# NVIDIA-ISAAC-ROS/isaac_ros_nvblox

Measured on NVIDIA H100. Metric: depth-frames/sec (TSDF+ESDF integrate, 640x480 @ 5 cm voxels), higher is better.
Workload: dtype f32

## Files before the change

### isaac_ros_nvblox_b200/csrc/nvb_api.cu

```cuda
#include <algorithm>
#include <array>
#include <cfloat>
#include <cmath>
#include <cstdio>
#include <cstring>
#include <functional>
#include <set>
#include <string>
#include <vector>

#include "nvb_internal.cuh"

using namespace nvb;

namespace {

thread_local std::string g_last_error;

int fail(int code, const std::string& msg) {
  g_last_error = msg;
  return code;
}

#define NVB_CUDA(expr)                                                                               \
// ... 992 lines not shown
      launchEsdfSliceAllocateAndMark(c, from_tracker ? nullptr : in_xyz_dev, todo.slots, todo.count,
                                     from_tracker ? upper : n_explicit, m->num_sms, st);
      m->launches += 3;
    } else {
      launchEsdfAllocate(c, from_tracker ? nullptr : in_xyz_dev, todo.slots, todo.count, from_tracker ? upper : n_explicit, st);
      launchEsdfMark(c, upper, m->num_sms, st);
      m->launches += 2;
    }
  };
  if (m->esdf_persistent) {
    cudaStream_t es = m->esdf_stream;
    NVB_CUDA(cudaEventRecord(m->esdf_ready, m->stream));
    NVB_CUDA(cudaStreamWaitEvent(es, m->esdf_ready, 0));
    beginStageOn(m, 3, es);
    allocAndMark(es);
    endStageOn(m, es);
    NVB_CUDA(cudaEventRecord(m->mark_done, es));
    NVB_CUDA(cudaStreamWaitEvent(m->stream, m->mark_done, 0));
    beginStageOn(m, 4, es);
    launchEsdfClear(c, m->esdf.capacity, m->num_sms, es);
    m->launches++;
    endStageOn(m, es);
    beginStageOn(m, 5, es);
    e = m->esdf_persistent == 3   ? launchEsdfComputeX(c, m->num_sms, m->esdf_reserved_sms, es, &launches)
        : m->esdf_persistent == 2 ? launchEsdfComputeGes(c, m->num_sms, es, &launches)
                                  : launchEsdfComputePersistent(c, m->num_sms, es, &launches);
    endStageOn(m, es);
    if (e == cudaSuccess) {
      NVB_CUDA(cudaEventRecord(m->esdf_done, es));
      m->esdf_in_flight = true;
    }
  } else {
    NVB_CUDA(joinEsdf(m));
    beginStage(m, 3);
    allocAndMark(m->stream);
    endStage(m);
    beginStage(m, 4);
    launchEsdfClear(c, m->esdf.capacity, m->num_sms, m->stream);
    m->launches++;
    endStage(m);
    beginStage(m, 5);
    e = runEsdfComputeHostLoop(c, m->num_sms, m->stream, &launches);
    endStage(m);
  }
  m->launches += launches;
  if (e != cudaSuccess) return fail(NVB_ERR_CUDA, std::string("ESDF compute launch: ") + cudaGetErrorString(e));
  return NVB_OK;
}

}

extern "C" {

const char* nvb_last_error(void) { return g_last_error.c_str(); }
const char* nvb_version(void) { return "nvblox_b200 0.1 (sm_90a)"; }

int32_t nvb_device_count(void) {
  int n = 0;
  if (cudaGetDeviceCount(&n) != cudaSuccess) {
    cudaGetLastError();
    return 0;
  }
  return n;
}

void nvb_default_mapper_options(NvbMapperOptions* o) {
  if (!o) return;
  o->voxel_size_m = 0.05f;
  o->device = 0;
  o->tsdf_capacity_blocks = kDefaultCapacity;
  o->esdf_capacity_blocks = kDefaultCapacity;
  o->esdf_persistent = 3;
  o->projective_layer_type = NVB_PROJECTIVE_TSDF;
  o->keep_last_view = 0;
}
void nvb_default_tsdf_params(NvbTsdfParams* p) {
  if (!p) return;
  memset(p, 0, sizeof(*p));
  p->truncation_distance_vox = 4.0f;
  p->max_integration_distance_m = 7.0f;
  p->max_weight = 5.0f;
  p->invalid_depth_decay_factor = -1.0f;
  p->weighting_type = NVB_WEIGHT_INVERSE_SQUARE;
  p->raycast_subsampling = 4;
  p->workspace_bounds_type = NVB_WS_UNBOUNDED;
}
void nvb_default_esdf_params(NvbEsdfParams* p) {
  if (!p) return;
  p->max_esdf_distance_m = 2.0f;
  p->max_site_distance_vox = 1.0f;
  p->min_weight = 1e-4f;
  p->occupied_threshold = 0.5f;
}
void nvb_default_occupancy_params(NvbOccupancyParams* p) {
  if (!p) return;
  p->free_region_occupancy_probability = 0.3f;
  p->occupied_region_occupancy_probability = 0.7f;
  p->unobserved_region_occupancy_probability = 0.5f;
  p->occupied_region_half_width_m = 0.1f;
}

static int createMapperResources(const NvbMapperOptions* opts, NvbMapper* m) {
  m->device = opts->device;
  cudaDeviceProp prop;
  NVB_CUDA(cudaGetDeviceProperties(&prop, opts->device));
  m->num_sms = prop.multiProcessorCount;
  m->voxel_size = opts->voxel_size_m;
  m->block_size = opts->voxel_size_m * (float)kVps;
  nvb_default_tsdf_params(&m->tp);
  nvb_default_esdf_params(&m->ep);
  nvb_default_occupancy_params(&m->op);
  nvb_default_tsdf_decay_params(&m->tdp);
  nvb_default_occupancy_decay_params(&m->odp);
  nvb_default_freespace_params(&m->fp);
  nvb_default_esdf_slice_params(&m->sp);
  nvb_default_color_params(&m->cp);
  nvb_default_ground_plane_params(&m->gp);
  m->projective_layer_type = opts->projective_layer_type;
  m->keep_last_view = opts->keep_last_view ? 1 : 0;
  m->esdf_persistent = opts->esdf_persistent;
  m->esdf_split_min_k = esdfWaveXSplitMinK();
  if (const char* e = getenv("NVB_GES_SWITCH")) m->ges_switch = atoi(e);
  {
    const char* e = getenv("NVB_CLEAR_PRUNE");
    m->prune_default = m->esdf_persistent == 3 && !(e && atoi(e) == 0);
    m->prune_ok = m->prune_default;
  }
  NVB_CUDA(cudaStreamCreateWithFlags(&m->stream, cudaStreamNonBlocking));
  NVB_CUDA(cudaStreamCreateWithFlags(&m->copy_stream, cudaStreamNonBlocking));
  {
    int lo = 0, hi = 0;
    cudaDeviceGetStreamPriorityRange(&lo, &hi);
    NVB_CUDA(cudaStreamCreateWithPriority(&m->esdf_stream, cudaStreamNonBlocking, hi));
  }
  NVB_CUDA(cudaEventCreateWithFlags(&m->esdf_ready, cudaEventDisableTiming));
  NVB_CUDA(cudaEventCreateWithFlags(&m->esdf_done, cudaEventDisableTiming));
  NVB_CUDA(cudaEventCreateWithFlags(&m->mark_done, cudaEventDisableTiming));
  const int tcap = opts->tsdf_capacity_blocks > 0 ? opts->tsdf_capacity_blocks : kDefaultCapacity;
  const int ecap = std::max(opts->esdf_capacity_blocks > 0 ? opts->esdf_capacity_blocks : kDefaultCapacity, tcap);
  int rc;
  if ((rc = allocLayer(&m->tsdf, tcap, m->projective_layer_type == NVB_PROJECTIVE_OCCUPANCY ? kOccBlockBytes : kTsdfBlockBytes,
                       m->stream))) return rc;
  if ((rc = allocLayer(&m->esdf, ecap, kEsdfBlockBytes, m->stream))) return rc;
  if (m->projective_layer_type == NVB_PROJECTIVE_TSDF_WITH_FREESPACE &&
      (rc = allocLayer(&m->freespace, tcap, kFreespaceBlockBytes, m->stream)))
    return rc;
  NVB_CUDA(m->esdf_ints.grow(m, kNumInts, kNumInts, 0));
  if ((rc = growTracker(m, tcap))) return rc;
  if ((rc = allocEsdfScratch(m, ecap))) return rc;
  const int one = 1;
  NVB_CUDA(cudaMemcpyAsync(m->esdf_ints.get() + kRingId, &one, sizeof(int), cudaMemcpyHostToDevice, m->stream));
  m->frame_count = m->esdf_ints.get() + kFrameCount;
  m->error_dev = m->esdf_ints.get() + kError;
  NVB_CUDA(m->clr_bits.grow(m, 2048, 2048));
  NVB_CUDA(m->stats.grow(m, 16, 16, 0));
  NVB_CUDA(m->phase_max.grow(m, 4000, 4000, 0));
  NVB_CUDA(m->barrier.grow(m, 16, 16, 0));
  NVB_CUDA(m->ticket.grow(m, 16, 16, 0));
  NVB_CUDA(cudaMallocHost(&m->h_ints, 64 * sizeof(int)));
  memset(m->h_ints, 0, 64 * sizeof(int));
  NVB_CUDA(cudaMallocHost(&m->h_list, (size_t)kHostListCap * sizeof(int4)));
  NVB_CUDA(cudaMallocHost(&m->h_count_ring, kCountRing * sizeof(int)));
  for (int k = 0; k < kCountRing; k++) {
    NVB_CUDA(cudaEventCreateWithFlags(&m->count_events[k], cudaEventDisableTiming));
    m->count_pending[k] = false;
    m->count_cum_at[k] = 0;
  }
  for (int k = 0; k < kStagingBuffers; k++) {
    NVB_CUDA(cudaEventCreateWithFlags(&m->stage_copied[k], cudaEventDisableTiming));
    NVB_CUDA(cudaEventCreateWithFlags(&m->stage_consumed[k], cudaEventDisableTiming));
  }
  NVB_CUDA(syncAll(m));
  return NVB_OK;
}

int32_t nvb_mapper_create(const NvbMapperOptions* opts, NvbMapper** out) {
  if (!opts || !out) return fail(NVB_ERR_INVALID_ARGUMENT, "null argument");
  if (!(opts->voxel_size_m > 0.0f)) return fail(NVB_ERR_INVALID_ARGUMENT, "voxel_size_m must be > 0");
  int ndev = 0;
  if (cudaGetDeviceCount(&ndev) != cudaSuccess || ndev == 0) {
    cudaGetLastError();
    return fail(NVB_ERR_NO_DEVICE, "no CUDA device: the depth-integration path has no CPU fallback");
  }
  if (opts->device < 0 || opts->device >= ndev) return fail(NVB_ERR_INVALID_ARGUMENT, "bad device ordinal");
  if (opts->projective_layer_type != NVB_PROJECTIVE_TSDF && opts->projective_layer_type != NVB_PROJECTIVE_OCCUPANCY &&
      opts->projective_layer_type != NVB_PROJECTIVE_TSDF_WITH_FREESPACE)
    return fail(NVB_ERR_INVALID_ARGUMENT, "unknown projective_layer_type");
  NVB_CUDA(cudaSetDevice(opts->device));
  NvbMapper* m = new NvbMapper();
  const int rc = createMapperResources(opts, m);
  if (rc != NVB_OK) {
    const std::string why = g_last_error;
    nvb_mapper_destroy(m);
    cudaGetLastError();
    g_last_error = why;
    return rc;
  }
  *out = m;
  return NVB_OK;
}

void nvb_mapper_destroy(NvbMapper* m) {
  if (!m) return;
  cudaSetDevice(m->device);
  syncAll(m);
  cudaStreamSynchronize(m->copy_stream);
  collectStages(m);
  cudaEventDestroy(m->esdf_ready), cudaEventDestroy(m->esdf_done), cudaEventDestroy(m->mark_done);
  cudaStreamDestroy(m->esdf_stream);
  freeLayer(&m->tsdf), freeLayer(&m->esdf);
  if (m->freespace.blocks) freeLayer(&m->freespace);
  if (m->color.blocks) freeLayer(&m->color);
  for (int k = 0; k < kStagingBuffers; k++) {
    cudaEventDestroy(m->stage_copied[k]), cudaEventDestroy(m->stage_consumed[k]);
  }
  if (m->dyn_event) cudaEventDestroy(m->dyn_event);
  if (m->query_event) cudaEventDestroy(m->query_event);
  if (m->mesh.blocks) freeLayer(&m->mesh);
  cudaFreeHost(m->h_ints), cudaFreeHost(m->h_count_ring), cudaFreeHost(m->h_list);
  for (int k = 0; k < kCountRing; k++) cudaEventDestroy(m->count_events[k]);
  cudaStreamDestroy(m->stream), cudaStreamDestroy(m->copy_stream);
  delete m;
}

static int resetLayers(NvbMapper* m) {
  NVB_CUDA(syncAll(m));
  std::vector<DevLayer*> layers = {&m->tsdf, &m->esdf};
  if (m->freespace.blocks) layers.push_back(&m->freespace);
  if (m->color.blocks) layers.push_back(&m->color);
  for (DevLayer* L : layers) {
    int count = 0;
    NVB_CUDA(cudaMemcpy(&count, L->count, sizeof(int), cudaMemcpyDeviceToHost));
    count = std::min(count, L->capacity);
    NVB_CUDA(cudaMemsetAsync(L->blocks, 0, (size_t)count * L->block_bytes, m->stream));
    NVB_CUDA(cudaMemsetAsync(L->count, 0, sizeof(int), m->stream));
    NVB_CUDA(cudaMemsetAsync(L->free_count, 0, sizeof(int), m->stream));
    launchFillU64(L->hash.keys, kEmptyKey, (size_t)L->hash.mask + 1, m->stream);
  }
  int rc;
  if ((rc = resetTracker(m))) return rc;
  NVB_CUDA(cudaMemsetAsync(m->esdf_ints.get() + kClearedCount, 0, sizeof(int), m->stream));
  NVB_CUDA(cudaMemsetAsync(m->esdf_ints.get() + kClearedSeq, 0, sizeof(int), m->stream));
  NVB_CUDA(cudaMemsetAsync(m->esdf_ints.get() + kDeadClearedCount, 0, sizeof(int), m->stream));
  NVB_CUDA(cudaMemsetAsync(m->seed_upd.get(), 0, (size_t)m->esdf.capacity * sizeof(int), m->stream));
  NVB_CUDA(cudaMemsetAsync(m->seed_clr.get(), 0, (size_t)m->esdf.capacity * sizeof(int), m->stream));
  NVB_CUDA(cudaMemsetAsync(m->psum.get(), 0, 2 * (size_t)m->esdf.capacity * sizeof(int), m->stream));
  m->prune_ok = m->prune_default;
  NVB_CUDA(cudaMemsetAsync(m->nbr.get(), 0xFE, (size_t)m->esdf.capacity * 6 * sizeof(int), m->stream));
  NVB_CUDA(cudaMemsetAsync(m->nbr27.get(), 0xFE, (size_t)m->esdf.capacity * 27 * sizeof(int), m->stream));
  NVB_CUDA(cudaMemsetAsync(m->error_dev, 0, sizeof(int), m->stream));
  if (m->mesh.blocks) {
    NVB_CUDA(cudaMemsetAsync(m->mesh.blocks, 0, (size_t)m->mesh.capacity * m->mesh.block_bytes, m->stream));
    NVB_CUDA(cudaMemsetAsync(m->mesh.count, 0, sizeof(int), m->stream));
    NVB_CUDA(cudaMemsetAsync(m->mesh.free_count, 0, sizeof(int), m->stream));
    launchFillU64(m->mesh.hash.keys, kEmptyKey, (size_t)m->mesh.hash.mask + 1, m->stream);
    NVB_CUDA(cudaMemsetAsync(m->mesh_state.get(), 0, kArenaInts * sizeof(int), m->stream));
  }
  m->tsdf_count_ub = 0, m->tsdf_count_confirmed = 0, m->esdf_extra_ub = 0;
  m->cells_cum = 0, m->confirmed_cum = 0;
  for (int k = 0; k < kCountRing; k++) m->count_pending[k] = false;
  NVB_CUDA(syncAll(m));
  return NVB_OK;
}

int32_t nvb_mapper_clear(NvbMapper* m) {
  if (!m) return fail(NVB_ERR_INVALID_ARGUMENT, "null mapper");
  NVB_CUDA(cudaSetDevice(m->device));
  const int rc = resetLayers(m);
  if (rc) return rc;
  m->esdf_mode = 0;
  m->fs_last_update_ms = 0;
  m->has_last_view = false;
  return NVB_OK;
}

int32_t nvb_mapper_set_tsdf_params(NvbMapper* m, const NvbTsdfParams* p) {
  if (!m || !p) return fail(NVB_ERR_INVALID_ARGUMENT, "null argument");
  if (!(p->max_weight > 0.0f)) return fail(NVB_ERR_INVALID_ARGUMENT, "max_weight must be > 0");
  if (!(p->truncation_distance_vox > 0.0f)) return fail(NVB_ERR_INVALID_ARGUMENT, "truncation_distance_vox must be > 0");
  if (p->raycast_subsampling < 1) return fail(NVB_ERR_INVALID_ARGUMENT, "raycast_subsampling must be >= 1");
  if (p->weighting_type < 0 || p->weighting_type > NVB_WEIGHT_LINEAR_WITH_MAX)
    return fail(NVB_ERR_INVALID_ARGUMENT, "unknown weighting_type");
  if (p->workspace_bounds_type < 0 || p->workspace_bounds_type > NVB_WS_BOUNDING_BOX)
    return fail(NVB_ERR_INVALID_ARGUMENT, "unknown workspace_bounds_type");
  m->tp = *p;
  return NVB_OK;
}
int32_t nvb_mapper_get_tsdf_params(const NvbMapper* m, NvbTsdfParams* p) {
  if (!m || !p) return fail(NVB_ERR_INVALID_ARGUMENT, "null argument");
  *p = m->tp;
  return NVB_OK;
}
int32_t nvb_mapper_set_esdf_params(NvbMapper* m, const NvbEsdfParams* p) {
  if (!m || !p) return fail(NVB_ERR_INVALID_ARGUMENT, "null argument");
  if (!(p->max_esdf_distance_m > 0.0f) || !(p->max_site_distance_vox > 0.0f) || !(p->min_weight > 0.0f))
    return fail(NVB_ERR_INVALID_ARGUMENT, "ESDF parameters must be > 0");
  if (!(p->occupied_threshold >= 0.0f && p->occupied_threshold <= 1.0f))
    return fail(NVB_ERR_INVALID_ARGUMENT, "occupied_threshold must be a probability");
  m->ep = *p;
  return NVB_OK;
}
int32_t nvb_mapper_get_esdf_params(const NvbMapper* m, NvbEsdfParams* p) {
  if (!m || !p) return fail(NVB_ERR_INVALID_ARGUMENT, "null argument");
  *p = m->ep;
  return NVB_OK;
}
int32_t nvb_mapper_set_occupancy_params(NvbMapper* m, const NvbOccupancyParams* p) {
// ... 2306 lines not shown
```

### isaac_ros_nvblox_b200/csrc/nvb_esdf.cu

```cuda
#include "nvb_esdf_common.cuh"
#include "nvb_tma.cuh"

#include <cstdlib>

namespace nvb {

namespace {

constexpr int kClearBitWords = 2048;
__device__ __forceinline__ int clearBitWord(int x, int y) { return ((x & 63) << 5) | (y & 31); }

__device__ __forceinline__ void resetEsdfUpdate(const EsdfCtx& c, int n) {
  const int i = blockIdx.x * blockDim.x + threadIdx.x;
  if (i == 0) {
    *c.work_count = n;
    *c.upd_count = 0;
    *c.clr_count = 0;
    c.clr_aabb[0] = c.clr_aabb[1] = c.clr_aabb[2] = INT32_MAX;
    c.clr_aabb[3] = c.clr_aabb[4] = c.clr_aabb[5] = INT32_MIN;
    c.ring_count[0] = c.ring_count[1] = 0;
    c.ring_count[2] = 0;
    c.ges_counts[0] = c.ges_counts[1] = c.ges_counts[2] = c.ges_counts[3] = 0;
    *c.barrier = 0;
    for (int k = 0; k < 16; k++) c.stats[k] = 0;
    c.stats[0] = n;
  }
  for (int q = i; q < 4000; q += gridDim.x * blockDim.x) c.phase_max[q] = 0ull;
  if (c.clr_bits)
    for (int q = i; q < kClearBitWords; q += gridDim.x * blockDim.x) c.clr_bits[q] = 0u;
}

__global__ void esdfAllocateKernel(EsdfCtx c, const int* in_xyz, const int* in_slots, const int* in_count_dev,
                                   int in_count_host) {
  const int n = in_count_dev ? *in_count_dev : in_count_host;
  const int i = blockIdx.x * blockDim.x + threadIdx.x;
  resetEsdfUpdate(c, n);
  if (i >= n) return;
  int x, y, z, tslot;
  if (in_slots) {
    tslot = in_slots[i];
    if (c.tracker_dirty) c.tracker_dirty[tslot] = 0;
    x = c.tsdf.block_index[3 * tslot], y = c.tsdf.block_index[3 * tslot + 1], z = c.tsdf.block_index[3 * tslot + 2];
  } else {
    x = in_xyz[3 * i], y = in_xyz[3 * i + 1], z = in_xyz[3 * i + 2];
    tslot = hashFind(c.tsdf.hash, x, y, z);
  }
  bool was_new;
  const int eslot = hashFindOrInsert(c.esdf, x, y, z, c.error, &was_new);
  const int fslot = c.use_freespace ? hashFind(c.freespace.hash, x, y, z) : -1;
  c.work[i] = make_int4(eslot, tslot, was_new ? 1 : 0, fslot);
}

constexpr int kMarkLocalMax = 64;
struct MarkLocal {
  int upd[kMarkLocalMax];
  int clr[kMarkLocalMax];
  int nu, nc;
  int aabb[6];
};
__device__ __forceinline__ void markLocalInit(MarkLocal& ml) {
  ml.nu = ml.nc = 0;
  ml.aabb[0] = ml.aabb[1] = ml.aabb[2] = INT32_MAX;
  ml.aabb[3] = ml.aabb[4] = ml.aabb[5] = INT32_MIN;
}
__device__ __forceinline__ void markLocalFlush(const EsdfCtx& c, MarkLocal& ml) {
  if (ml.nu) {
    const int base = atomicAdd(c.upd_count, ml.nu);
    for (int i = 0; i < ml.nu; i++) c.upd_list[base + i] = ml.upd[i];
  }
  if (ml.nc) {
    const int base = atomicAdd(c.clr_count, ml.nc);
    for (int i = 0; i < ml.nc; i++) c.clr_list[base + i] = ml.clr[i];
    atomicMin(c.clr_aabb + 0, ml.aabb[0]), atomicMin(c.clr_aabb + 1, ml.aabb[1]), atomicMin(c.clr_aabb + 2, ml.aabb[2]);
    atomicMax(c.clr_aabb + 3, ml.aabb[3]), atomicMax(c.clr_aabb + 4, ml.aabb[4]), atomicMax(c.clr_aabb + 5, ml.aabb[5]);
  }
  markLocalInit(ml);
}
__device__ __forceinline__ void markLocalRecord(const EsdfCtx& c, MarkLocal& ml, int slot, bool updated, bool cleared,
                                                const int* bi_known = nullptr) {
  if (updated) {
    if (ml.nu == kMarkLocalMax) markLocalFlush(c, ml);
    ml.upd[ml.nu++] = slot;
    c.seed_upd[slot] = c.update_seq;
  }
  if (cleared) {
    if (ml.nc == kMarkLocalMax) markLocalFlush(c, ml);
    ml.clr[ml.nc++] = slot;
    const int* bi = bi_known ? bi_known : c.esdf.block_index + 3 * slot;
    const int x = bi[0], y = bi[1], z = bi[2];
    ml.aabb[0] = min(ml.aabb[0], x), ml.aabb[1] = min(ml.aabb[1], y), ml.aabb[2] = min(ml.aabb[2], z);
    ml.aabb[3] = max(ml.aabb[3], x), ml.aabb[4] = max(ml.aabb[4], y), ml.aabb[5] = max(ml.aabb[5], z);
    if (c.clr_bits) atomicOr(c.clr_bits + clearBitWord(x, y), 1u << (z & 31));
  }
}

__device__ __forceinline__ void updatePersistentClearedList(const EsdfCtx& c, int nclr) {
  if (nclr > 0) {
    *c.cleared_count = 0;
    *c.cleared_seq = c.update_seq;
    if (c.dead_cleared_count) *c.dead_cleared_count = 0;
    return;
  }
  if (!c.dead_cleared_count) return;
  int nd = *c.dead_cleared_count;
  for (int i = 0; i < nd;) {
    const int slot = hashFind(c.esdf.hash, c.dead_cleared_xyz[3 * i], c.dead_cleared_xyz[3 * i + 1], c.dead_cleared_xyz[3 * i + 2]);
    if (slot >= 0) {
      c.cleared_list[(*c.cleared_count)++] = slot;
      c.seed_clr[slot] = *c.cleared_seq;
      nd--;
      c.dead_cleared_xyz[3 * i] = c.dead_cleared_xyz[3 * nd], c.dead_cleared_xyz[3 * i + 1] = c.dead_cleared_xyz[3 * nd + 1],
                          c.dead_cleared_xyz[3 * i + 2] = c.dead_cleared_xyz[3 * nd + 2];
    } else {
      i++;
    }
  }
  *c.dead_cleared_count = nd;
}

__device__ __forceinline__ int markBegin(const EsdfCtx& c, MarkLocal& ml) {
  if (threadIdx.x == 0) markLocalInit(ml);
  const int n = *c.work_count;
  if (blockIdx.x == 0 && threadIdx.x == 0 && c.tracker_todo_count) *c.tracker_todo_count = 0;
  return n;
}

__device__ __forceinline__ void markFinish(const EsdfCtx& c, MarkLocal& ml) {
  markLocalFlush(c, ml);
  __threadfence();
  if (atomicAdd(c.ring_count + 2, 1) == (int)gridDim.x - 1) {
    __threadfence();
    const int nclr = *(volatile int*)c.clr_count;
    const int nupd = *(volatile int*)c.upd_count;
    updatePersistentClearedList(c, nclr);
    c.stats[1] = nupd, c.stats[2] = nclr;
  }
}

__device__ __forceinline__ bool updateVoxelToChanges(unsigned int* e, bool is_observed, bool is_inside, bool is_site,
                                                     float max_sq, bool& updated, bool& cleared) {
  float sq = __uint_as_float(e[0]);
  int p0 = (int)e[1], p1 = (int)e[2], p2 = (int)e[3];
  const unsigned int fl = e[4];
  bool e_inside = flagInside(fl), e_observed = flagObserved(fl), e_site = flagSite(fl);
  if (is_observed) {
    if (e_inside && !is_inside) {
      p0 = p1 = p2 = 0, sq = max_sq, e_site = false;
      cleared = true;
    }
    e_inside = is_inside;
    if (is_site) {
      if (!e_site) e_site = true, sq = 0.0f, p0 = p1 = p2 = 0;
      updated = true;
    } else if (e_site) {
      p0 = p1 = p2 = 0, sq = max_sq, e_site = false;
      cleared = true;
    } else if (!e_observed) {
      p0 = p1 = p2 = 0, sq = max_sq, e_site = false;
    } else if ((double)sq <= 1e-4) {
      p0 = p1 = p2 = 0, sq = max_sq, e_site = false;
      cleared = true;
    }
    e_observed = true;
  } else {
    p0 = p1 = p2 = 0, sq = max_sq, e_site = false;
    cleared = true;
    e_observed = false;
  }
  const unsigned int nfl = (fl & 0xff000000u) | (e_inside ? 1u : 0u) | (e_observed ? 0x100u : 0u) | (e_site ? 0x10000u : 0u);
  const unsigned int nsq = __float_as_uint(sq);
  if (nsq == e[0] && (unsigned)p0 == e[1] && (unsigned)p1 == e[2] && (unsigned)p2 == e[3] && nfl == fl) return false;
  e[0] = nsq, e[1] = (unsigned)p0, e[2] = (unsigned)p1, e[3] = (unsigned)p2, e[4] = nfl;
  return true;
}

struct TsdfSite {
  using Voxel = float2;
  static constexpr int kBlockBytes = kTsdfBlockBytes;
  float min_weight, max_site_distance_m;
  __device__ static TsdfSite of(const EsdfCtx& c) { return {c.min_weight, c.max_site_distance_m}; }
  __device__ static float value(float2 t) { return t.x; }
  __device__ bool observed(float2 t) const { return t.y >= min_weight; }
  __device__ bool inside(float d) const { return d <= 0.0f; }
  __device__ bool nearSurface(float d) const { return fabsf(d) <= max_site_distance_m; }
  __device__ float squashInit(float max_sq) const { return 2.0f * max_sq; }
  __device__ float squash(float acc, float d) const { return fminf(acc, d); }
};
struct OccupancySite {
  using Voxel = float;
  static constexpr int kBlockBytes = kOccBlockBytes;
  float occupied_threshold_log_odds;
  __device__ static OccupancySite of(const EsdfCtx& c) { return {c.occupied_threshold_log_odds}; }
  __device__ static float value(float lo) { return lo; }
  __device__ bool observed(float lo) const { return fabsf(lo - 0.0f) > 1e-4f; }
  __device__ bool inside(float lo) const { return lo > occupied_threshold_log_odds; }
  __device__ bool nearSurface(float) const { return true; }
  __device__ float squashInit(float) const { return 0.0f; }
  __device__ float squash(float acc, float lo) const { return fmaxf(acc, lo); }
};

template <class Site>
__device__ __forceinline__ bool markVoxel(const Site& site, unsigned int* e, typename Site::Voxel t, bool is_freespace,
                                          float max_sq, bool& updated, bool& cleared) {
  const float d = Site::value(t);
  const bool is_inside = site.inside(d) & !is_freespace;
  return updateVoxelToChanges(e, site.observed(t), is_inside, is_inside && site.nearSurface(d), max_sq, updated, cleared);
}

template <class Site>
__device__ __forceinline__ void markStaged(const EsdfCtx& c, const Site site) {
  using V = typename Site::Voxel;
  __shared__ __align__(16) unsigned int s[kBlockWords];
  __shared__ int s_flags[3];
  __shared__ MarkLocal ml;
  const int tid = threadIdx.x;
  const int n = markBegin(c, ml);
  for (int item = blockIdx.x; item < n; item += gridDim.x) {
    const int4 w = c.work[item];
    if (w.x >= 0 && w.z) linkNewBlock(c, w.x, tid);
    if (w.x < 0 || w.y < 0) continue;
    if (tid < 3) s_flags[tid] = 0;
    uint4* gblk = reinterpret_cast<uint4*>(esdfBlockPtr(c.esdf, w.x));
    for (int k = tid; k < kBlockWords / 4; k += kThreads) reinterpret_cast<uint4*>(s)[k] = gblk[k];
    const V* src = reinterpret_cast<const V*>(c.tsdf.blocks + (size_t)w.y * Site::kBlockBytes);
    const V t0 = src[tid], t1 = src[tid + kThreads];
    const bool fs0 = isVoxelFreespace(c.freespace, w.w, tid), fs1 = isVoxelFreespace(c.freespace, w.w, tid + kThreads);
    __syncthreads();
    bool updated = false, cleared = false, changed = false;
#pragma unroll
    for (int h = 0; h < 2; h++)
      changed |= markVoxel(site, s + (tid + h * kThreads) * kEsdfVoxelWords, h ? t1 : t0, h ? fs1 : fs0, c.max_sq, updated,
                           cleared);
    if (updated) s_flags[0] = 1;
    if (cleared) s_flags[1] = 1;
    if (changed) s_flags[2] = 1;
    __syncthreads();
    if (s_flags[2]) {
      for (int k = tid; k < kBlockWords / 4; k += kThreads) gblk[k] = reinterpret_cast<uint4*>(s)[k];
    }
    if (tid == 0) markLocalRecord(c, ml, w.x, s_flags[0] != 0, s_flags[1] != 0);
    __syncthreads();
  }
  if (tid == 0) markFinish(c, ml);
}
__global__ void __launch_bounds__(kThreads, 5) esdfMarkKernel(EsdfCtx c) { markStaged(c, TsdfSite::of(c)); }
__global__ void __launch_bounds__(kThreads, 5) esdfMarkOccupancyKernel(EsdfCtx c) { markStaged(c, OccupancySite::of(c)); }

constexpr int kMarkStages = 3;
struct __align__(128) MarkStage {
  unsigned int esdf[kBlockWords];
  float2 tsdf[kVpb];
};
constexpr unsigned int kMarkStageTxBytes = kEsdfBlockBytes + kTsdfBlockBytes;

__global__ void __launch_bounds__(kThreads) esdfMarkTmaKernel(EsdfCtx c) {
  extern __shared__ __align__(128) unsigned char smem_raw[];
  MarkStage* st = reinterpret_cast<MarkStage*>(smem_raw);
  __shared__ __align__(8) uint64_t s_bar[kMarkStages];
  __shared__ int4 s_work[kMarkStages];
  __shared__ int s_flags[3];
  __shared__ int s_bi[3];
  __shared__ MarkLocal ml;
  const int tid = threadIdx.x;
  const int n = markBegin(c, ml);
  const int my_count = (n > (int)blockIdx.x) ? (n - (int)blockIdx.x + (int)gridDim.x - 1) / (int)gridDim.x : 0;
  if (tid == 0) {
    for (int s = 0; s < kMarkStages; s++) tma::mbarInit(&s_bar[s], 1);
    tma::fenceBarrierInit();
  }
  __syncthreads();
  auto issue = [&](int j) {
    const int s = j % kMarkStages;
    const int4 w = c.work[blockIdx.x + j * gridDim.x];
    s_work[s] = w;
    if (w.x >= 0 && w.y >= 0) {
      tma::mbarArriveExpectTx(&s_bar[s], kMarkStageTxBytes);
      tma::bulkLoad(st[s].esdf, c.esdf.blocks + (size_t)w.x * kEsdfBlockBytes, kEsdfBlockBytes, &s_bar[s]);
      tma::bulkLoad(st[s].tsdf, c.tsdf.blocks + (size_t)w.y * kTsdfBlockBytes, kTsdfBlockBytes, &s_bar[s]);
    } else {
      tma::mbarArrive(&s_bar[s]);
    }
  };
  if (tid == 0) {
    for (int j = 0; j < kMarkStages - 1 && j < my_count; j++) issue(j);
  }
  __syncthreads();
  for (int j = 0; j < my_count; j++) {
    const int s = j % kMarkStages;
    if (tid == 0 && j + kMarkStages - 1 < my_count) {
      tma::bulkWaitRead<0>();
      issue(j + kMarkStages - 1);
    }
    tma::mbarWait(&s_bar[s], (unsigned int)((j / kMarkStages) & 1));
    const int4 w = s_work[s];
    if (tid >= 32 && tid < 35 && w.x >= 0) s_bi[tid - 32] = c.esdf.block_index[3 * w.x + (tid - 32)];
    if (w.x >= 0 && w.z) linkNewBlock(c, w.x, tid);
    const bool valid = (w.x >= 0 && w.y >= 0);
    if (tid < 3) s_flags[tid] = 0;
    __syncthreads();
    if (valid) {
      unsigned int* sblk = st[s].esdf;
      bool updated = false, cleared = false, changed = false;
#pragma unroll
      for (int h = 0; h < 2; h++) {
        const float2 t = st[s].tsdf[tid + h * kThreads];
        unsigned int* e = sblk + (tid + h * kThreads) * kEsdfVoxelWords;
        float sq = __uint_as_float(e[0]);
        int p0 = (int)e[1], p1 = (int)e[2], p2 = (int)e[3];
        const unsigned int fl = e[4];
        bool e_inside = flagInside(fl), e_observed = flagObserved(fl), e_site = flagSite(fl);
        const bool is_observed = t.y >= c.min_weight;
        if (is_observed) {
          const bool is_inside = t.x <= 0.0f;
          const bool is_site = is_inside && (fabsf(t.x) <= c.max_site_distance_m);
          if (e_inside && !is_inside) {
            p0 = p1 = p2 = 0, sq = c.max_sq, e_site = false;
            cleared = true;
          }
          e_inside = is_inside;
          if (is_site) {
            if (!e_site) {
              e_site = true, sq = 0.0f, p0 = p1 = p2 = 0;
            }
            updated = true;
          } else {
            if (e_site) {
              p0 = p1 = p2 = 0, sq = c.max_sq, e_site = false;
              cleared = true;
            } else if (!e_observed) {
              p0 = p1 = p2 = 0, sq = c.max_sq, e_site = false;
            } else if ((double)sq <= 1e-4) {
              p0 = p1 = p2 = 0, sq = c.max_sq, e_site = false;
              cleared = true;
            }
          }
          e_observed = true;
        } else {
          p0 = p1 = p2 = 0, sq = c.max_sq, e_site = false;
          cleared = true;
          e_observed = false;
        }
        const unsigned int nfl = (fl & 0xff000000u) | (e_inside ? 1u : 0u) | (e_observed ? 0x100u : 0u) |
                                 (e_site ? 0x10000u : 0u);
        const unsigned int nsq = __float_as_uint(sq);
        if (nsq != e[0] || (unsigned)p0 != e[1] || (unsigned)p1 != e[2] || (unsigned)p2 != e[3] || nfl != fl) {
          e[0] = nsq, e[1] = (unsigned)p0, e[2] = (unsigned)p1, e[3] = (unsigned)p2, e[4] = nfl;
          changed = true;
        }
      }
      if (updated) s_flags[0] = 1;
      if (cleared) s_flags[1] = 1;
      if (changed) s_flags[2] = 1;
      tma::fenceProxyAsyncShared();
    }
    __syncthreads();
    if (valid && tid == 0) {
      if (s_flags[2]) {
        tma::bulkStore(c.esdf.blocks + (size_t)w.x * kEsdfBlockBytes, st[s].esdf, kEsdfBlockBytes);
        tma::bulkCommit();
      }
      markLocalRecord(c, ml, w.x, s_flags[0] != 0, s_flags[1] != 0, s_bi);
    }
    __syncthreads();
  }
  if (tid == 0) {
    tma::bulkWait<0>();
    markFinish(c, ml);
  }
}

constexpr int kClearMaxCand = 256;
__device__ __forceinline__ void clearPrefetch(const EsdfCtx& c, unsigned int* sblk, int* snb, int slot, int tid) {
  const unsigned char* g = c.esdf.blocks + (size_t)slot * kEsdfBlockBytes;
  for (int k = tid; k < kBlockWords / 4; k += kThreads) {
    const unsigned int d = (unsigned int)__cvta_generic_to_shared(sblk + 4 * k);
    asm volatile("cp.async.cg.shared.global [%0], [%1], 16;" ::"r"(d), "l"(g + 16 * k) : "memory");
  }
  if (tid < 27) {
    const unsigned int d = (unsigned int)__cvta_generic_to_shared(snb + tid);
    asm volatile("cp.async.ca.shared.global [%0], [%1], 4;" ::"r"(d), "l"(c.nbr27 + 27 * slot + tid) : "memory");
  }
  asm volatile("cp.async.commit_group;" ::: "memory");
}

__global__ void __launch_bounds__(kThreads) esdfClearKernel(EsdfCtx c) {
  __shared__ __align__(16) unsigned int s_blk[2][kBlockWords];
  __shared__ int s_nb[2][32];
  __shared__ int s_cand[kClearMaxCand];
  __shared__ int s_done[kClearMaxCand];
  __shared__ int s_ncand, s_ndone, s_any;
  const int nclr = *c.clr_count;
  if (nclr == 0) return;
  const int tid = threadIdx.x, lane = tid & 31;
  const int nblocks = *c.esdf.count < c.esdf.capacity ? *c.esdf.count : c.esdf.capacity;
  const float bs = c.block_size;
  float amin[3], amax[3];
  int ia[3], ib[3];
#pragma unroll
  for (int a = 0; a < 3; a++) {
    ia[a] = c.clr_aabb[a], ib[a] = c.clr_aabb[3 + a];
    amin[a] = (float)ia[a] * bs;
    amax[a] = ((float)ib[a] + 1.0f) * bs;
  }
  const bool use_bits = c.prune && c.clr_bits != nullptr;
  long long ncand_total = 0, nread_total = 0;
  for (long long first = (long long)blockIdx.x; first < (long long)nblocks; first += (long long)gridDim.x * kThreads) {
    if (tid == 0) s_ncand = 0, s_ndone = 0;
    __syncthreads();
    const long long slot_ll = first + (long long)tid * gridDim.x;
    bool is_cand = false, ref_cand = false;
    if (slot_ll < nblocks && c.esdf.block_index[3 * slot_ll] != kDeadSlotX) {
      const int* bi = c.esdf.block_index + 3 * slot_ll;
      const int b3[3] = {bi[0], bi[1], bi[2]};
      float d2 = 0.0f;
#pragma unroll
      for (int a = 0; a < 3; a++) {
        const float lo = (float)b3[a] * bs, hi = ((float)b3[a] + 1.0f) * bs;
        if (amin[a] > hi) {
          const float aux = amin[a] - hi;
          d2 += aux * aux;
        } else if (lo > amax[a]) {
          const float aux = lo - amax[a];
          d2 += aux * aux;
        }
      }
      is_cand = !(sqrtf(d2) > c.max_esdf_distance_m);
      if (is_cand && c.prune) {
        const uint2 pw = __ldg(reinterpret_cast<const uint2*>(c.psum) + slot_ll);
        if (pw.x == 0u && pw.y == 0u) {
          is_cand = false, ref_cand = true;
        } else if (pw.x != 0xffffffffu && pw.y != 0xffffffffu) {
          ref_cand = true;
          int lo[3], hi[3];
          bool hit = true;
#pragma unroll
          for (int a = 0; a < 3; a++) {
            int l = 99, h = -99;
            if (pw.x) l = (int)((pw.x >> (10 * a)) & 31u) - 16, h = (int)((pw.x >> (10 * a + 5)) & 31u) - 16;
            if (pw.y) l = min(l, (int)((pw.y >> (10 * a)) & 31u) - 16), h = max(h, (int)((pw.y >> (10 * a + 5)) & 31u) - 16);
            lo[a] = b3[a] + l, hi[a] = b3[a] + h;
            lo[a] = lo[a] > ia[a] ? lo[a] : ia[a], hi[a] = hi[a] < ib[a] ? hi[a] : ib[a];
            hit = hit && lo[a] <= hi[a];
          }
          if (hit && use_bits) {
            unsigned int zmask = 0xffffffffu;
            if (hi[2] - lo[2] < 31) {
              const unsigned int m = (1u << (hi[2] - lo[2] + 1)) - 1u;
              const int sh = lo[2] & 31;
              zmask = (m << sh) | (sh ? (m >> (32 - sh)) : 0u);
            }
            hit = false;
            for (int x = lo[0]; x <= hi[0] && !hit; x++)
              for (int y = lo[1]; y <= hi[1]; y++)
                if (__ldg(c.clr_bits + clearBitWord(x, y)) & zmask) {
                  hit = true;
                  break;
                }
          }
          is_cand = hit;
        }
      }
      ref_cand = ref_cand || is_cand;
    }
    const unsigned int ref_ballot = __ballot_sync(0xffffffffu, ref_cand);
    const unsigned int ballot = __ballot_sync(0xffffffffu, is_cand);
    int wbase = 0;
    if (lane == 0 && ballot) wbase = atomicAdd(&s_ncand, __popc(ballot));
    wbase = __shfl_sync(0xffffffffu, wbase, 0);
    if (is_cand) s_cand[wbase + __popc(ballot & ((1u << lane) - 1u))] = (int)slot_ll;
    if (lane == 0) ncand_total += __popc(ref_ballot);
    __syncthreads();
    const int ncand = s_ncand;
    if (tid == 0) nread_total += ncand;
    if (ncand > 0) clearPrefetch(c, s_blk[0], s_nb[0], s_cand[0], tid);
    for (int i = 0; i < ncand; i++) {
      const int buf = i & 1;
      const int slot = s_cand[i];
      if (i + 1 < ncand) {
        clearPrefetch(c, s_blk[buf ^ 1], s_nb[buf ^ 1], s_cand[i + 1], tid);
        asm volatile("cp.async.wait_group 1;" ::: "memory");
      } else {
        asm volatile("cp.async.wait_group 0;" ::: "memory");
      }
      if (tid == 0) s_any = 0;
      __syncthreads();
      const unsigned int* s = s_blk[buf];
      const int* nbrow = s_nb[buf];
      unsigned int* gw = esdfBlockPtr(c.esdf, slot);
      const int bx = c.esdf.block_index[3 * slot], by = c.esdf.block_index[3 * slot + 1], bz = c.esdf.block_index[3 * slot + 2];
      bool any = false;
#pragma unroll
      for (int h = 0; h < 2; h++) {
        const int v = tid + h * kThreads;
        const unsigned int* e = s + v * kEsdfVoxelWords;
        const unsigned int fl = e[4];
        const int p[3] = {(int)e[1], (int)e[2], (int)e[3]};
        if (flagObserved(fl) && !flagSite(fl) && (p[0] != 0 || p[1] != 0 || p[2] != 0)) {
          const int vi[3] = {v >> 6, (v >> 3) & 7, v & 7};
          int nb[3], nv[3];
#pragma unroll
          for (int a = 0; a < 3; a++) {
            const int q = vi[a] + p[a];
            nb[a] = q >> 3;
            nv[a] = q & (kVps - 1);
          }
          const int pv = (nv[0] * kVps + nv[1]) * kVps + nv[2];
          bool parent_is_site = false;
          if (nb[0] == 0 && nb[1] == 0 && nb[2] == 0) {
            parent_is_site = flagSite(s[pv * kEsdfVoxelWords + 4]);
          } else {
            int ps = -2;
            if (nb[0] >= -1 && nb[0] <= 1 && nb[1] >= -1 && nb[1] <= 1 && nb[2] >= -1 && nb[2] <= 1)
              ps = nbrow[(nb[0] + 1) * 9 + (nb[1] + 1) * 3 + (nb[2] + 1)];
            if (ps < -1) ps = hashFind(c.esdf.hash, bx + nb[0], by + nb[1], bz + nb[2]);
            if (ps >= 0) parent_is_site = flagSite(__ldcg(esdfBlockPtr(c.esdf, ps) + pv * kEsdfVoxelWords + 4));
          }
          if (!parent_is_site) {
            unsigned int* g = gw + v * kEsdfVoxelWords;
            g[0] = __float_as_uint(c.max_sq), g[1] = 0u, g[2] = 0u, g[3] = 0u;
            any = true;
          }
        }
      }
      if (any) s_any = 1;
      __syncthreads();
      if (tid == 0 && s_any) {
        s_done[s_ndone++] = slot;
        c.seed_clr[slot] = c.update_seq;
      }
    }
    __syncthreads();
    if (s_ndone > 0) {
      __shared__ int s_base;
      if (tid == 0) s_base = atomicAdd(c.cleared_count, s_ndone);
      __syncthreads();
      for (int i = tid; i < s_ndone; i += kThreads) c.cleared_list[s_base + i] = s_done[i];
    }
    __syncthreads();
  }
  if (lane == 0 && ncand_total) atomicAdd((unsigned long long*)&c.stats[3], (unsigned long long)ncand_total);
  if (tid == 0 && nread_total) atomicAdd((unsigned long long*)&c.stats[13], (unsigned long long)nread_total);
}


__device__ __forceinline__ bool sweepLine(unsigned int* s, int c0, int c1, int c2, int axis, float max_sq) {
  const int stride = (axis == 0) ? 64 : ((axis == 1) ? 8 : 1);
  const int basev = c0 * 64 + c1 * 8 + c2;
  bool changed = false;
#pragma unroll
  for (int pass = 0; pass < 2; pass++) {
    int l0 = 0, l1 = 0, l2 = 0;
    bool found = false;
#pragma unroll
    for (int k = 0; k < kVps; k++) {
      const int cc = pass ? (kVps - 1 - k) : k;
      unsigned int* e = s + (basev + cc * stride) * kEsdfVoxelWords;
      const unsigned int fl = e[4];
      if (!flagObserved(fl)) continue;
      const int v0 = (axis == 0) ? cc : c0, v1 = (axis == 1) ? cc : c1, v2 = (axis == 2) ? cc : c2;
      if (flagSite(fl)) {
        l0 = v0, l1 = v1, l2 = v2;
        found = true;
      } else if (!found) {
        if (__uint_as_float(e[0]) < max_sq) {
          found = true;
          l0 = (int)e[1] + v0, l1 = (int)e[2] + v1, l2 = (int)e[3] + v2;
        }
      } else {
        const int d0 = l0 - v0, d1 = l1 - v1, d2 = l2 - v2;
        const float pdist = (float)(d0 * d0 + (d1 * d1 + d2 * d2));
        const float sq = __uint_as_float(e[0]);
        if (sq > pdist) {
          e[1] = (unsigned)d0, e[2] = (unsigned)d1, e[3] = (unsigned)d2;
          e[0] = __float_as_uint(pdist);
          changed = true;
        } else if (sq < max_sq) {
          l0 = (int)e[1] + v0, l1 = (int)e[2] + v1, l2 = (int)e[3] + v2;
        }
      }
    }
  }
  return changed;
}

__device__ void phaseSweep(const EsdfCtx& c, const int* src, int* list, int n, int* stamp, int ring,
                           unsigned int* smem, int* s_changed, int cta, int nctas) {
  const int tid = threadIdx.x, group = tid >> 6, lane64 = tid & 63;
  unsigned int* sm = smem + group * kBlockWords;
  const int a = lane64 >> 3, b = lane64 & 7;
  for (int base = cta * kGroups; base < n; base += nctas * kGroups) {
    const int item = base + group;
    int slot = -1;
    if (item < n) {
      slot = src ? __ldcg(src + item) : __ldcg(list + item);
      if (src && lane64 == 0) {
        list[item] = slot;
        stamp[slot] = ring;
      }
    }
    if (lane64 == 0) s_changed[group] = 0;
    if (slot >= 0) loadBlockGroup(sm, esdfBlockPtr(c.esdf, slot), lane64);
    __syncthreads();
    bool ch = false;
    if (slot >= 0) ch |= sweepLine(sm, 0, a, b, 0, c.max_sq);
    __syncthreads();
    if (slot >= 0) ch |= sweepLine(sm, a, 0, b, 1, c.max_sq);
    __syncthreads();
    if (slot >= 0) ch |= sweepLine(sm, a, b, 0, 2, c.max_sq);
    if (ch) s_changed[group] = 1;
    __syncthreads();
    if (slot >= 0 && s_changed[group]) storeBlockGroup(esdfBlockPtr(c.esdf, slot), sm, lane64);
    __syncthreads();
  }
}

__device__ __forceinline__ void appendUnique(int slot, int* nxt, int* nxt_count, int* stamp_nxt, int ring_next) {
  if (atomicExch(stamp_nxt + slot, ring_next) != ring_next) nxt[atomicAdd(nxt_count, 1)] = slot;
}

__device__ void phaseNeighbors(const EsdfCtx& c, int axis, const int* cur, int n, const int* stamp_cur, int ring,
                               int* nxt, int* nxt_count, int* stamp_nxt, int* s_slot, int* s_upd, int cta,
                               int nctas) {
  const int tid = threadIdx.x, group = tid >> 6, lane64 = tid & 63;
  const int entry_in_cta = group >> 1, side = group & 1;
  const int u = lane64 >> 3, w = lane64 & 7;
  const int strideA = (axis == 0) ? 64 : ((axis == 1) ? 8 : 1);
  const int faceBase = (axis == 0) ? (u * 8 + w) : ((axis == 1) ? (u * 64 + w) : (u * 64 + w * 8));
  const int vHi = faceBase + (kVps - 1) * strideA, vLo = faceBase;
  for (int base = cta * (kGroups / 2); base < n; base += nctas * (kGroups / 2)) {
    const int item = base + entry_in_cta;
    if (lane64 == 0) {
      int other = -1;
      int mine = -1;
      if (item < n) {
        mine = __ldcg(cur + item);
        const int* bi = c.esdf.block_index + 3 * mine;
        int x = bi[0], y = bi[1], z = bi[2];
        const int d = side ? -1 : 1;
        if (axis == 0) x += d;
        else if (axis == 1) y += d;
        else z += d;
        other = hashFind(c.esdf.hash, x, y, z);
      }
      s_slot[group * 2] = mine;
      s_slot[group * 2 + 1] = other;
      s_upd[group * 2] = 0;
      s_upd[group * 2 + 1] = 0;
    }
    __syncthreads();
    const int mine = s_slot[group * 2], other = s_slot[group * 2 + 1];
    if (mine >= 0 && other >= 0) {
      const bool other_member = (__ldcg(stamp_cur + other) == ring);
      if (side == 0) {
        unsigned int* gA = esdfBlockPtr(c.esdf, mine) + vHi * kEsdfVoxelWords;
        unsigned int* gB = esdfBlockPtr(c.esdf, other) + vLo * kEsdfVoxelWords;
        VoxelRegs A = loadVoxel(gA), B = loadVoxel(gB);
        if (updateSingleNeighbor(A, B, gB, axis, +1, c.max_sq)) s_upd[group * 2 + 1] = 1;
        if (other_member) {
          if (updateSingleNeighbor(B, A, gA, axis, -1, c.max_sq)) s_upd[group * 2] = 1;
        }
      } else if (!other_member) {
        unsigned int* gA = esdfBlockPtr(c.esdf, other) + vHi * kEsdfVoxelWords;
        unsigned int* gB = esdfBlockPtr(c.esdf, mine) + vLo * kEsdfVoxelWords;
        VoxelRegs A = loadVoxel(gA), B = loadVoxel(gB);
        if (updateSingleNeighbor(B, A, gA, axis, -1, c.max_sq)) s_upd[group * 2 + 1] = 1;
      }
    }
    __syncthreads();
    if (lane64 == 0 && mine >= 0 && other >= 0) {
      if (s_upd[group * 2]) appendUnique(mine, nxt, nxt_count, stamp_nxt, ring + 1);
      if (s_upd[group * 2 + 1]) appendUnique(other, nxt, nxt_count, stamp_nxt, ring + 1);
    }
    __syncthreads();
  }
}

__global__ void __launch_bounds__(kThreads) esdfSweepKernel(EsdfCtx c, const int* src, int* list, const int* n_dev,
                                                            int* stamp, int ring) {
  extern __shared__ __align__(16) unsigned int smem[];
  __shared__ int s_changed[kGroups];
  phaseSweep(c, src, list, *n_dev, stamp, ring, smem, s_changed, blockIdx.x, gridDim.x);
}
__global__ void __launch_bounds__(kThreads) esdfNeighborKernel(EsdfCtx c, int axis, const int* cur, const int* n_dev,
                                                               const int* stamp_cur, int ring, int* nxt,
                                                               int* nxt_count, int* stamp_nxt) {
  __shared__ int s_slot[kGroups * 2];
  __shared__ int s_upd[kGroups * 2];
  phaseNeighbors(c, axis, cur, *n_dev, stamp_cur, ring, nxt, nxt_count, stamp_nxt, s_slot, s_upd, blockIdx.x,
                 gridDim.x);
}
__global__ void esdfSetIntKernel(int* p, int v) { *p = v; }

constexpr size_t kSweepSmemBytes = (size_t)kGroups * kEsdfBlockBytes;

// ... 320 lines not shown
```

Baseline: 3150.

## Add x-column occupancy bitmap and paired hash probes to ESDF clear kernel

Adds a second level to the cleared-block bitmap: a per-x word marks which y columns hold cleared blocks, so candidate selection visits only set y bits instead of scanning every y in the range. The clear kernel's per-voxel parent lookup is split into phases, and the two voxels per thread probe the hash table together so their memory latencies overlap. The clear kernel also gets a min-blocks launch bound of 5, and disabled-by-default profiling counters are added. The cost is one extra atomicOr per cleared block and more register state in the clear loop.

```diff
diff --git a/isaac_ros_nvblox_b200/csrc/nvb_api.cu b/isaac_ros_nvblox_b200/csrc/nvb_api.cu
--- a/isaac_ros_nvblox_b200/csrc/nvb_api.cu
+++ b/isaac_ros_nvblox_b200/csrc/nvb_api.cu
@@ -1168,7 +1168,7 @@
   NVB_CUDA(cudaMemcpyAsync(m->esdf_ints.get() + kRingId, &one, sizeof(int), cudaMemcpyHostToDevice, m->stream));
   m->frame_count = m->esdf_ints.get() + kFrameCount;
   m->error_dev = m->esdf_ints.get() + kError;
-  NVB_CUDA(m->clr_bits.grow(m, 2048, 2048));
+  NVB_CUDA(m->clr_bits.grow(m, 2048 + 64, 2048 + 64));
   NVB_CUDA(m->stats.grow(m, 16, 16, 0));
   NVB_CUDA(m->phase_max.grow(m, 4000, 4000, 0));
   NVB_CUDA(m->barrier.grow(m, 16, 16, 0));
diff --git a/isaac_ros_nvblox_b200/csrc/nvb_esdf.cu b/isaac_ros_nvblox_b200/csrc/nvb_esdf.cu
--- a/isaac_ros_nvblox_b200/csrc/nvb_esdf.cu
+++ b/isaac_ros_nvblox_b200/csrc/nvb_esdf.cu
@@ -3,12 +3,32 @@
 
 #include <cstdlib>
 
+#ifndef NVB_PREPASS_PROF
+#define NVB_PREPASS_PROF 0
+#endif
+
 namespace nvb {
 
 namespace {
 
+constexpr bool kProf = NVB_PREPASS_PROF != 0;
+constexpr int kPP = 3900;
+__device__ __forceinline__ void profAdd(const EsdfCtx& c, int k, unsigned long long v) {
+  if (kProf && v) atomicAdd(c.phase_max + kPP + k, v);
+}
+__device__ __forceinline__ void profMax(const EsdfCtx& c, int k, unsigned long long v) {
+  if (kProf) atomicMax(c.phase_max + kPP + k, v);
+}
+
 constexpr int kClearBitWords = 2048;
+constexpr int kClearColumnWords = 64;
 __device__ __forceinline__ int clearBitWord(int x, int y) { return ((x & 63) << 5) | (y & 31); }
+__device__ __forceinline__ unsigned int foldedRangeMask(int lo, int hi) {
+  if (hi - lo >= 31) return 0xffffffffu;
+  const unsigned int m = (1u << (hi - lo + 1)) - 1u;
+  const int sh = lo & 31;
+  return (m << sh) | (sh ? (m >> (32 - sh)) : 0u);
+}
 
 __device__ __forceinline__ void resetEsdfUpdate(const EsdfCtx& c, int n) {
   const int i = blockIdx.x * blockDim.x + threadIdx.x;
@@ -27,7 +47,7 @@
   }
   for (int q = i; q < 4000; q += gridDim.x * blockDim.x) c.phase_max[q] = 0ull;
   if (c.clr_bits)
-    for (int q = i; q < kClearBitWords; q += gridDim.x * blockDim.x) c.clr_bits[q] = 0u;
+    for (int q = i; q < kClearBitWords + kClearColumnWords; q += gridDim.x * blockDim.x) c.clr_bits[q] = 0u;
 }
 
 __global__ void esdfAllocateKernel(EsdfCtx c, const int* in_xyz, const int* in_slots, const int* in_count_dev,
@@ -90,7 +110,10 @@
     const int x = bi[0], y = bi[1], z = bi[2];
     ml.aabb[0] = min(ml.aabb[0], x), ml.aabb[1] = min(ml.aabb[1], y), ml.aabb[2] = min(ml.aabb[2], z);
     ml.aabb[3] = max(ml.aabb[3], x), ml.aabb[4] = max(ml.aabb[4], y), ml.aabb[5] = max(ml.aabb[5], z);
-    if (c.clr_bits) atomicOr(c.clr_bits + clearBitWord(x, y), 1u << (z & 31));
+    if (c.clr_bits) {
+      atomicOr(c.clr_bits + clearBitWord(x, y), 1u << (z & 31));
+      atomicOr(c.clr_bits + kClearBitWords + (x & 63), 1u << (y & 31));
+    }
   }
 }
 
@@ -262,6 +285,9 @@
   __shared__ int s_bi[3];
   __shared__ MarkLocal ml;
   const int tid = threadIdx.x;
+  const long long t_start = kProf ? clock64() : 0;
+  long long t_wait = 0;
+  int n_wb = 0, n_valid = 0;
   const int n = markBegin(c, ml);
   const int my_count = (n > (int)blockIdx.x) ? (n - (int)blockIdx.x + (int)gridDim.x - 1) / (int)gridDim.x : 0;
   if (tid == 0) {
@@ -291,7 +317,9 @@
       tma::bulkWaitRead<0>();
       issue(j + kMarkStages - 1);
     }
+    const long long t_w0 = kProf ? clock64() : 0;
     tma::mbarWait(&s_bar[s], (unsigned int)((j / kMarkStages) & 1));
+    if (kProf) t_wait += clock64() - t_w0;
     const int4 w = s_work[s];
     if (tid >= 32 && tid < 35 && w.x >= 0) s_bi[tid - 32] = c.esdf.block_index[3 * w.x + (tid - 32)];
     if (w.x >= 0 && w.z) linkNewBlock(c, w.x, tid);
@@ -360,14 +388,47 @@
         tma::bulkCommit();
       }
       markLocalRecord(c, ml, w.x, s_flags[0] != 0, s_flags[1] != 0, s_bi);
+      n_valid++, n_wb += s_flags[2] ? 1 : 0;
     }
     __syncthreads();
   }
   if (tid == 0) {
     tma::bulkWait<0>();
     markFinish(c, ml);
-  }
-}
+    if (kProf) {
+      const long long t_all = clock64() - t_start;
+      if (blockIdx.x == 0) profAdd(c, 0, gridDim.x);
+      profMax(c, 1, my_count), profAdd(c, 2, n_wb), profAdd(c, 3, n_valid);
+      profAdd(c, 4, t_wait), profAdd(c, 5, t_all - t_wait), profMax(c, 6, t_wait), profMax(c, 7, t_all);
+    }
+  }
+}
+
+__device__ __forceinline__ void hashFindPair(const DevHash& h, bool f0, int x0, int y0, int z0, bool f1, int x1, int y1, int z1,
+                                             int& r0, int& r1) {
+  bool a0 = f0 && indexInRange(x0, y0, z0), a1 = f1 && indexInRange(x1, y1, z1);
+  if (f0 && !a0) r0 = -1;
+  if (f1 && !a1) r1 = -1;
+  const unsigned long long key0 = packIndex(x0, y0, z0), key1 = packIndex(x1, y1, z1);
+  unsigned int p0 = hashKey(key0) & h.mask, p1 = hashKey(key1) & h.mask;
+  while (a0 || a1) {
+    unsigned long long k0 = 0ull, k1 = 0ull;
+    int v0 = -1, v1 = -1;
+    if (a0) k0 = h.keys[p0], v0 = h.vals[p0];
+    if (a1) k1 = h.keys[p1], v1 = h.vals[p1];
+    if (a0) {
+      if (k0 == key0) r0 = v0, a0 = false;
+      else if (k0 == kEmptyKey) r0 = -1, a0 = false;
+      else p0 = (p0 + 1) & h.mask;
+    }
+    if (a1) {
+      if (k1 == key1) r1 = v1, a1 = false;
+      else if (k1 == kEmptyKey) r1 = -1, a1 = false;
+      else p1 = (p1 + 1) & h.mask;
+    }
+  }
+}
+constexpr int kOwnBlock = -3;
 
 constexpr int kClearMaxCand = 256;
 __device__ __forceinline__ void clearPrefetch(const EsdfCtx& c, unsigned int* sblk, int* snb, int slot, int tid) {
@@ -383,7 +444,24 @@
   asm volatile("cp.async.commit_group;" ::: "memory");
 }
 
-__global__ void __launch_bounds__(kThreads) esdfClearKernel(EsdfCtx c) {
+__device__ __forceinline__ void clearProfFinish(const EsdfCtx& c, long long t_start, long long t_sel, long long t_cwait,
+                                                long long t_cproc, int ncand, const unsigned int* lk_n,
+                                                const unsigned int* lk_cyc, unsigned int lk_in_clr) {
+  for (int k = 0; k < 3; k++) {
+    const unsigned int site = __reduce_add_sync(0xffffffffu, lk_n[k] & 0xffffu), other = __reduce_add_sync(0xffffffffu, lk_n[k] >> 16);
+    const unsigned int cyc = __reduce_add_sync(0xffffffffu, lk_cyc[k]);
+    if ((threadIdx.x & 31) == 0) profAdd(c, 25 + k, site), profAdd(c, 28 + k, other), profAdd(c, 31 + k, cyc);
+  }
+  const unsigned int in_clr = __reduce_add_sync(0xffffffffu, lk_in_clr);
+  if ((threadIdx.x & 31) == 0) profAdd(c, 34, in_clr);
+  if (threadIdx.x != 0) return;
+  if (blockIdx.x == 0) profAdd(c, 10, gridDim.x);
+  profAdd(c, 11, t_sel), profMax(c, 12, t_sel), profMax(c, 13, ncand), profAdd(c, 24, ncand);
+  profAdd(c, 14 + (ncand <= 4 ? ncand : ncand <= 6 ? 5 : ncand <= 8 ? 6 : 7), 1);
+  profAdd(c, 22, t_cwait), profAdd(c, 23, t_cproc), profMax(c, 35, clock64() - t_start);
+}
+
+__global__ void __launch_bounds__(kThreads, 5) esdfClearKernel(EsdfCtx c) {
   __shared__ __align__(16) unsigned int s_blk[2][kBlockWords];
   __shared__ int s_nb[2][32];
   __shared__ int s_cand[kClearMaxCand];
@@ -404,7 +482,11 @@
   }
   const bool use_bits = c.prune && c.clr_bits != nullptr;
   long long ncand_total = 0, nread_total = 0;
+  const long long t_start = kProf ? clock64() : 0;
+  long long t_sel = 0, t_cwait = 0, t_cproc = 0;
+  unsigned int lk_n[3] = {0, 0, 0}, lk_cyc[3] = {0, 0, 0}, lk_in_clr = 0;
   for (long long first = (long long)blockIdx.x; first < (long long)nblocks; first += (long long)gridDim.x * kThreads) {
+    const long long t_round = kProf ? clock64() : 0;
     if (tid == 0) s_ncand = 0, s_ndone = 0;
     __syncthreads();
     const long long slot_ll = first + (long long)tid * gridDim.x;
@@ -443,19 +525,16 @@
             hit = hit && lo[a] <= hi[a];
           }
           if (hit && use_bits) {
-            unsigned int zmask = 0xffffffffu;
-            if (hi[2] - lo[2] < 31) {
-              const unsigned int m = (1u << (hi[2] - lo[2] + 1)) - 1u;
-              const int sh = lo[2] & 31;
-              zmask = (m << sh) | (sh ? (m >> (32 - sh)) : 0u);
+            const unsigned int ymask = foldedRangeMask(lo[1], hi[1]), zmask = foldedRangeMask(lo[2], hi[2]);
+            hit = false;
+            for (int x = lo[0]; x <= hi[0] && !hit; x++) {
+              unsigned int ys = __ldg(c.clr_bits + kClearBitWords + (x & 63)) & ymask;
+              while (ys && !hit) {
+                const int y = __ffs(ys) - 1;
+                ys &= ys - 1u;
+                hit = (__ldg(c.clr_bits + (((x & 63) << 5) | y)) & zmask) != 0u;
+              }
             }
-            hit = false;
-            for (int x = lo[0]; x <= hi[0] && !hit; x++)
-              for (int y = lo[1]; y <= hi[1]; y++)
-                if (__ldg(c.clr_bits + clearBitWord(x, y)) & zmask) {
-                  hit = true;
-                  break;
-                }
           }
           is_cand = hit;
         }
@@ -472,10 +551,12 @@
     __syncthreads();
     const int ncand = s_ncand;
     if (tid == 0) nread_total += ncand;
+    if (kProf) t_sel += clock64() - t_round;
     if (ncand > 0) clearPrefetch(c, s_blk[0], s_nb[0], s_cand[0], tid);
     for (int i = 0; i < ncand; i++) {
       const int buf = i & 1;
       const int slot = s_cand[i];
+      const long long t_c0 = kProf ? clock64() : 0;
       if (i + 1 < ncand) {
         clearPrefetch(c, s_blk[buf ^ 1], s_nb[buf ^ 1], s_cand[i + 1], tid);
         asm volatile("cp.async.wait_group 1;" ::: "memory");
@@ -484,42 +565,66 @@
       }
       if (tid == 0) s_any = 0;
       __syncthreads();
+      const long long t_c1 = kProf ? clock64() : 0;
       const unsigned int* s = s_blk[buf];
       const int* nbrow = s_nb[buf];
       unsigned int* gw = esdfBlockPtr(c.esdf, slot);
       const int bx = c.esdf.block_index[3 * slot], by = c.esdf.block_index[3 * slot + 1], bz = c.esdf.block_index[3 * slot + 2];
-      bool any = false;
+      bool test[2] = {false, false};
+      int pv[2] = {0, 0}, ps[2] = {-1, -1}, q[2][3] = {{0, 0, 0}, {0, 0, 0}};
+      int kind[2] = {0, 0};
+      const long long t_l0 = kProf ? clock64() : 0;
 #pragma unroll
       for (int h = 0; h < 2; h++) {
         const int v = tid + h * kThreads;
         const unsigned int* e = s + v * kEsdfVoxelWords;
         const unsigned int fl = e[4];
         const int p[3] = {(int)e[1], (int)e[2], (int)e[3]};
-        if (flagObserved(fl) && !flagSite(fl) && (p[0] != 0 || p[1] != 0 || p[2] != 0)) {
-          const int vi[3] = {v >> 6, (v >> 3) & 7, v & 7};
-          int nb[3], nv[3];
+        test[h] = flagObserved(fl) && !flagSite(fl) && (p[0] != 0 || p[1] != 0 || p[2] != 0);
+        if (!test[h]) continue;
+        const int vi[3] = {v >> 6, (v >> 3) & 7, v & 7};
+        int nb[3], nv[3];
 #pragma unroll
-          for (int a = 0; a < 3; a++) {
-            const int q = vi[a] + p[a];
-            nb[a] = q >> 3;
-            nv[a] = q & (kVps - 1);
-          }
-          const int pv = (nv[0] * kVps + nv[1]) * kVps + nv[2];
-          bool parent_is_site = false;
-          if (nb[0] == 0 && nb[1] == 0 && nb[2] == 0) {
-            parent_is_site = flagSite(s[pv * kEsdfVoxelWords + 4]);
-          } else {
-            int ps = -2;
-            if (nb[0] >= -1 && nb[0] <= 1 && nb[1] >= -1 && nb[1] <= 1 && nb[2] >= -1 && nb[2] <= 1)
-              ps = nbrow[(nb[0] + 1) * 9 + (nb[1] + 1) * 3 + (nb[2] + 1)];
-            if (ps < -1) ps = hashFind(c.esdf.hash, bx + nb[0], by + nb[1], bz + nb[2]);
-            if (ps >= 0) parent_is_site = flagSite(__ldcg(esdfBlockPtr(c.esdf, ps) + pv * kEsdfVoxelWords + 4));
-          }
-          if (!parent_is_site) {
-            unsigned int* g = gw + v * kEsdfVoxelWords;
-            g[0] = __float_as_uint(c.max_sq), g[1] = 0u, g[2] = 0u, g[3] = 0u;
-            any = true;
-          }
+        for (int a = 0; a < 3; a++) {
+          const int qa = vi[a] + p[a];
+          nb[a] = qa >> 3;
+          nv[a] = qa & (kVps - 1);
+        }
+        pv[h] = (nv[0] * kVps + nv[1]) * kVps + nv[2];
+        q[h][0] = bx + nb[0], q[h][1] = by + nb[1], q[h][2] = bz + nb[2];
+        if (nb[0] == 0 && nb[1] == 0 && nb[2] == 0) {
+          ps[h] = kOwnBlock;
+        } else {
+          ps[h] = -2, kind[h] = 1;
+          if (nb[0] >= -1 && nb[0] <= 1 && nb[1] >= -1 && nb[1] <= 1 && nb[2] >= -1 && nb[2] <= 1)
+            ps[h] = nbrow[(nb[0] + 1) * 9 + (nb[1] + 1) * 3 + (nb[2] + 1)];
+          if (ps[h] < -1) kind[h] = 2;
+        }
+      }
+      hashFindPair(c.esdf.hash, kind[0] == 2, q[0][0], q[0][1], q[0][2], kind[1] == 2, q[1][0], q[1][1], q[1][2], ps[0], ps[1]);
+      unsigned int pfl[2] = {0u, 0u};
+#pragma unroll
+      for (int h = 0; h < 2; h++) {
+        if (!test[h]) continue;
+        if (ps[h] == kOwnBlock) pfl[h] = s[pv[h] * kEsdfVoxelWords + 4];
+        else if (ps[h] >= 0) pfl[h] = __ldcg(esdfBlockPtr(c.esdf, ps[h]) + pv[h] * kEsdfVoxelWords + 4);
+      }
+      bool any = false;
+#pragma unroll
+      for (int h = 0; h < 2; h++) {
+        if (!test[h]) continue;
+        const bool parent_is_site = flagSite(pfl[h]);
+        if (kProf) {
+          lk_n[kind[h]] += parent_is_site ? 1u : 0x10000u;
+          if (h == 1 || !test[1]) lk_cyc[max(kind[0], kind[1])] += (unsigned int)(clock64() - t_l0);
+          if (kind[h] && c.clr_bits && q[h][0] >= ia[0] && q[h][0] <= ib[0] && q[h][1] >= ia[1] && q[h][1] <= ib[1] &&
+              q[h][2] >= ia[2] && q[h][2] <= ib[2] && ((c.clr_bits[clearBitWord(q[h][0], q[h][1])] >> (q[h][2] & 31)) & 1u))
+            lk_in_clr++;
+        }
+        if (!parent_is_site) {
+          unsigned int* g = gw + (tid + h * kThreads) * kEsdfVoxelWords;
+          g[0] = __float_as_uint(c.max_sq), g[1] = 0u, g[2] = 0u, g[3] = 0u;
+          any = true;
         }
       }
       if (any) s_any = 1;
@@ -528,6 +633,10 @@
         s_done[s_ndone++] = slot;
         c.seed_clr[slot] = c.update_seq;
       }
+      if (kProf) {
+        const long long t_c2 = clock64();
+        t_cwait += t_c1 - t_c0, t_cproc += t_c2 - t_c1;
+      }
     }
     __syncthreads();
     if (s_ndone > 0) {
@@ -540,6 +649,7 @@
   }
   if (lane == 0 && ncand_total) atomicAdd((unsigned long long*)&c.stats[3], (unsigned long long)ncand_total);
   if (tid == 0 && nread_total) atomicAdd((unsigned long long*)&c.stats[13], (unsigned long long)nread_total);
+  if (kProf) clearProfFinish(c, t_start, t_sel, t_cwait, t_cproc, (int)nread_total, lk_n, lk_cyc, lk_in_clr);
 }
 
 
```

After: 3139, median of 6. No clear change (-0.4%).
